# 294coder/Dif-PAN

Measured on AMD Instinct MI355X. Metric: fused megapixels/sec at T=1000, WV3 64x64x8 tiles, higher is better.
Workload: dtype f32-class (f16x2 split); 1 GPU; WV3 pansharpening, batch 64 of 64x64x8 tiles per GPU, T=1000 DDPM p_sample, fp32; tiles_per_gpu=64, tiles_total=64, T=1000, model_evaluations=1000, sampler=ddpm, parallelism=tile-shard x1, launches_per_denoising_step=132

## Files before the change

dif-pan_amd/csrc/ddif_dev.h:

```cpp
#pragma once
#include <hip/hip_runtime.h>

#ifdef DDIF_EMU
typedef hipemu_f32x16 f32x16;
typedef hipemu_f32x4 f32x4;
#define DDIF_MFMA_32x32x2(a, b, c) hipemu_mfma_32x32x2((a), (b), (c))
#define DDIF_MFMA_16x16x4(a, b, c) hipemu_mfma_16x16x4((a), (b), (c))
static inline f32x16 ddif_mfma_bf16_emu(float4 a, float4 b, f32x16 c) {
    hipemu_u32x4 ua, ub;
    __builtin_memcpy(&ua, &a, 16);
    __builtin_memcpy(&ub, &b, 16);
    return hipemu_mfma_32x32x16_bf16(ua, ub, c);
}
#define DDIF_MFMA_32x32x16_BF16(a, b, c) ddif_mfma_bf16_emu((a), (b), (c))
static inline f32x16 ddif_mfma_f16_emu(float4 a, float4 b, f32x16 c) {
    hipemu_u32x4 ua, ub;
    __builtin_memcpy(&ua, &a, 16);
    __builtin_memcpy(&ub, &b, 16);
    return hipemu_mfma_32x32x16_f16(ua, ub, c);
}
#define DDIF_MFMA_32x32x16_F16(a, b, c) ddif_mfma_f16_emu((a), (b), (c))
#define DDIF_DYN_SMEM(name) char* name = hipemu::tctx().dyn_smem
#define DDIF_SCHED_FENCE() ((void)0)
#else
// ... 103 lines not shown
#endif
__device__ __forceinline__ void dd_split2_pair(float a, float b, unsigned* hi, unsigned* lo) {
#ifdef DDIF_EMU
    const unsigned ha = dd_f16_bits(a), hb = dd_f16_bits(b);
    *hi = ha | (hb << 16);
    *lo = dd_f16_bits(a - dd_f16_val(ha)) | (dd_f16_bits(b - dd_f16_val(hb)) << 16);
#else
    typedef float v2f __attribute__((ext_vector_type(2)));
    typedef _Float16 v2h __attribute__((ext_vector_type(2)));
    const v2f v = {a, b};
    const v2h H = __builtin_convertvector(v, v2h);
    const v2f r = {a - (float)H.x, b - (float)H.y};
    *hi = __builtin_bit_cast(unsigned, H);
    *lo = __builtin_bit_cast(unsigned, __builtin_convertvector(r, v2h));
#endif
}
__device__ __forceinline__ float dd_silu_scaled(float x, float inv_s) {
#ifdef DDIF_EMU
    return x * (1.0f / fmaf(exp2f(-1.4426950408889634f * x), inv_s, inv_s));
#else
    return x * __builtin_amdgcn_rcpf(fmaf(__builtin_amdgcn_exp2f(-1.4426950408889634f * x), inv_s, inv_s));
#endif
}

__device__ __forceinline__ int dd_late(int v) {
#if !defined(DDIF_EMU) && defined(__HIP_DEVICE_COMPILE__)
    asm volatile("" : "+v"(v));
#endif
    return v;
}
// ... 144 lines not shown
```

dif-pan_amd/csrc/ddif_lr.cpp:

```cpp
#include "ddif_plan.h"
#include "kernels_lr.h"
#include "kernels_attn.h"

namespace ddif {

namespace {
template <int KS, int MB, int PRO, int EPI, bool F16 = false, bool B1 = false, bool ROWS = false>
ConvVariant lr_variant1(const char* name) {
    ConvVariant v;
    v.fn = conv_lr_kernel<KS, MB, PRO, EPI, 0, F16, B1, ROWS>;
    using G = LrGeom<KS, MB, PRO, (EPI & EPI_COLST) != 0, F16, B1>;
    v.smem = G::smem;
    v.th = G::TH;
    v.tw = G::TW;
    v.nt = 32;
    v.nthr = 256;
    v.x3 = true;
    v.f16 = F16;
    v.b1 = B1;
    v.lr = true;
    v.name = name;
    return v;
}
template <int MB, bool F16>
ConvVariant lr_rows_for(int pro, int epi) {
    if (pro == PRO_GN_SILU && epi == 0) return lr_variant1<3, MB, PRO_GN_SILU, 0, F16, false, true>("lr3x3_gn_silu_rows");
    if (pro == PRO_GN_SILU && epi == EPI_RES) return lr_variant1<3, MB, PRO_GN_SILU, EPI_RES, F16, false, true>("lr3x3_gn_silu_res_rows");
    if (pro == PRO_NONE && epi == EPI_SILU) return lr_variant1<3, MB, PRO_NONE, EPI_SILU, F16, false, true>("lr3x3_silu_rows");
    if (pro == PRO_NONE && epi == 0) return lr_variant1<3, MB, PRO_NONE, 0, F16, false, true>("lr3x3_rows");
    if (pro == PRO_NONE && epi == EPI_RES) return lr_variant1<3, MB, PRO_NONE, EPI_RES, F16, false, true>("lr3x3_res_rows");
    return ConvVariant();
}
template <int MB>
ConvVariant lr_for(int ks, int pro, int epi, int math) {
#define LRV(KS, PRO, EPI, NAME) (math == MATH_F16X2 ? lr_variant1<KS, MB, PRO, EPI, true>(NAME) : (math == MATH_BF16X1 ? lr_variant1<KS, MB, PRO, EPI, false, true>(NAME) : lr_variant1<KS, MB, PRO, EPI, false>(NAME)))
    if (ks == 3) {
        if (pro == PRO_GN_SILU && epi == 0) return LRV(3, PRO_GN_SILU, 0, "lr3x3_gn_silu");
        if (pro == PRO_GN_SILU && epi == EPI_RES) return LRV(3, PRO_GN_SILU, EPI_RES, "lr3x3_gn_silu_res");
        if (pro == PRO_NONE && epi == EPI_SILU) return LRV(3, PRO_NONE, EPI_SILU, "lr3x3_silu");
        if (pro == PRO_NONE && epi == 0) return LRV(3, PRO_NONE, 0, "lr3x3");
        if (pro == PRO_NONE && epi == EPI_RES) return LRV(3, PRO_NONE, EPI_RES, "lr3x3_res");
    } else if (ks == 1) {
        if (pro == PRO_NONE && epi == EPI_FILM) return LRV(1, PRO_NONE, EPI_FILM, "lr1x1_film");
        if (pro == PRO_NONE && epi == EPI_RES) return LRV(1, PRO_NONE, EPI_RES, "lr1x1_res");
        if (pro == PRO_NONE && epi == 0) return LRV(1, PRO_NONE, 0, "lr1x1");
        if (pro == PRO_NONE && epi == EPI_COLST) return LRV(1, PRO_NONE, EPI_COLST, "lr1x1_colstats");
        if (pro == PRO_GN && epi == 0) return LRV(1, PRO_GN, 0, "lr1x1_gn");
        if (pro == PRO_GN_SILU && epi == 0) return LRV(1, PRO_GN_SILU, 0, "lr1x1_gn_silu");
        if (pro == PRO_COLSM && epi == 0)
            return math == MATH_BF16X1 ? lr_variant1<1, MB, PRO_COLSM, 0, false, true>("lr1x1_colsoftmax") : lr_variant1<1, MB, PRO_COLSM, 0, false>("lr1x1_colsoftmax");
    }
// ... 46 lines not shown
```

dif-pan_amd/csrc/ddif_net.h:

```cpp
#pragma once
#include <mutex>
#include <cmath>
#include <cstdarg>
#include <cstdint>
#include <cstdio>
#include <cstring>
#include <functional>
#include <map>
#include <memory>
#include <string>
#include <vector>

#include "../../include/ddif.h"
#include "../../include/ddif_testops.h"
#include "ddif_dev.h"

namespace ddif {

extern thread_local std::string g_err;
int fail(int code, const char* fmt, ...);

#define DDIF_HIPCHK(x)                                                                                      \
    do {                                                                                                    \
        hipError_t e__ = (x);                                                                               \
        if (e__ != hipSuccess)                                                                              \
            return ::ddif::fail(DDIF_ERR_HIP, "%s failed: %s (%s:%d)", #x, hipGetErrorString(e__), __FILE__, \
                                __LINE__);                                                                  \
    } while (0)

enum { PRO_NONE = 0, PRO_GN = 1, PRO_GN_SILU = 2, PRO_COLSM = 3, PRO_GN_DW = 4 };

enum LayerKind { L_STEM, L_ENC, L_DOWN, L_MID, L_DEC, L_UP };

struct Layer {
    LayerKind kind;
    int cin = 0, cout = 0, cx = 0, cskip = 0;
    bool attn = false;
    std::string p;
};

struct PackedConv {
    const float* w = nullptr;
    const float* w_x3 = nullptr;
    const float* w_f16 = nullptr;
    const float* w_b1 = nullptr;
// ... 74 lines not shown
```

dif-pan_amd/csrc/ddif_plan.cpp:

```cpp
#include "ddif_plan.h"
#include <algorithm>
#include "kernels_conv.h"
#include "kernels_misc.h"
#include "attn_args.h"
#include "quantile_args.h"
#include "kernels_lafuse.h"

namespace ddif {

ConvVariant get_conv_variant(int ks, int stride, int ups, int ck, int pro, int cfg, int vec, int epi, int math) {
    if (cfg == 20 || cfg == 21)
        return (stride == 1 && !ups && vec == 1) ? get_lr_variant(ks, cfg == 20 ? 2 : 4, pro, epi, (math == MATH_F16X2 && pro == PRO_COLSM) ? MATH_BF16X3 : math) : ConvVariant();
    if (ks == 1) return get_conv_variant_k1(stride, ups, ck, pro, cfg, vec, epi);
    if (ks == 3) return epi ? get_conv_variant_k3e(stride, ups, ck, pro, cfg, vec, epi) : get_conv_variant_k3(stride, ups, ck, pro, cfg, vec);
    return ConvVariant();
}

static int num_cus();
static int x3_enabled() { static const int v = env_int("DDIF_X3", 1); return v; }
static int f16_enabled() { static const int v = env_int("DDIF_F16", 1); return v; }
int g_math_mode = [] { const char* e = getenv("DDIF_MATH"); return (e && std::strcmp(e, "bf16") == 0) ? 1 : 0; }();
int g_f16_raw = env_flag("DDIF_F16_RAW", true);
static int lr_rows_enabled() { static const int v = env_int("DDIF_LR_ROWS", 1); return v; }
static int lafuse_enabled() { static const int v = env_int("DDIF_LAFUSE", 1); return v; }
// ... 225 lines not shown
        allocs.push_back(q);
        bytes_allocated += arena_bytes;
        arena = reinterpret_cast<char*>(q);
    }
    if (int e = build_impl()) return e;
    if (arena_next != (int)lives.size()) return fail(DDIF_ERR_STATE, "plan arena: the two build passes disagree");
    return 0;
}

static int raise_dynamic_lds(ConvKernelFn fn, size_t var_smem) {
    if (var_smem + 8192 > 64 * 1024)
        DDIF_HIPCHK(hipFuncSetAttribute(reinterpret_cast<const void*>(fn), hipFuncAttributeMaxDynamicSharedMemorySize, (int)(var_smem + 8192)));
    return 0;
}

int Plan::add_conv(std::vector<Op>& prog, const ConvSpec& s, Tensor* out) {
    const PackedConv& pc = *s.pc;
    const int Hin = s.in0.H, Win = s.in0.W;
    const int Hc = s.ups ? 2 * Hin : Hin, Wc = s.ups ? 2 * Win : Win;
    const int Hout = s.stride == 2 ? (Hc - 1) / 2 + 1 : Hc, Wout = s.stride == 2 ? (Wc - 1) / 2 + 1 : Wc;
    const int c0 = s.in0.C, c1 = s.in1.C;
    if (c0 + c1 != pc.cin) return fail(DDIF_ERR_INVALID, "%s: input channels %d+%d != weight cin %d", s.name, c0, c1, pc.cin);
    if (pc.ks == 1 && (s.stride != 1 || s.ups)) return fail(DDIF_ERR_INVALID, "%s: 1x1 conv with stride/upsample", s.name);
    const int vec = (c0 % 4 != 0 || c1 % 4 != 0) ? 0 : ((c1 == 0 || c0 % pc.ck == 0) ? 1 : 2);
    if ((size_t)B * Hin * Win * (c0 > c1 ? c0 : c1) * 4 >= ((size_t)1 << 32) || (size_t)B * Hout * Wout * pc.cout * 8 >= ((size_t)1 << 32))
        return fail(DDIF_ERR_INVALID, "%s: a tensor of this batch reaches 4 GiB (32-bit offsets); split the batch", s.name);
    bool f16ok = f16_enabled() && !train_mode && pc.w_f16 && !s.w_override && !s.exact;
    const bool raw_in = !(s.pro == PRO_GN || s.pro == PRO_GN_SILU || s.pro == PRO_GN_DW);
    if (raw_in && !f16_raw) f16ok = false;
    if (f16ok && (s.pro == PRO_GN || s.pro == PRO_GN_SILU)) {
        auto ig = net->vec_absmax.find(s.gamma), ib = net->vec_absmax.find(s.beta);
// ... 31 lines not shown
    if (!var.fn && b1ok) {
        f16ok = f16ok0;
        choose(true, f16ok, false);
        var = variant(cfg, epi);
        general_kernel_if_no_lr(f16ok, false);
    }
    if (!var.fn) return fail(DDIF_ERR_INVALID, "%s: no kernel variant (ks=%d stride=%d ups=%d ck=%d pro=%d cfg=%d vec=%d epi=%d)", s.name, pc.ks, s.stride, s.ups, pc.ck, s.pro, cfg, vec, epi);
    bool lr_rows = false;
    if (var.lr && !var.b1 && pc.ks == 3 && Win == var.tw && Wout == Win && Hout == Hin && lr_rows_enabled()) {
        const ConvVariant vr = get_lr_variant(3, cfg == 20 ? 2 : 4, s.pro, epi, var.f16 ? MATH_F16X2 : MATH_BF16X3, true);
        if (vr.fn && vr.smem == var.smem) {
            var = vr;
            lr_rows = true;
        }
    }
    bool xf = false;
    if (s.xf && !train_mode && xf_enabled() && var.f16 && !var.lr && pc.ks == 3 && pc.cout == 32 && !s.ups && s.tb_off < 0 && !s.samp && s.xf->pc && s.xf->w && s.xf->film &&
        s.xf->pc->cin == 32 && s.xf->pc->bias && (s.xf->pc->cout == 32 || s.xf->pc->cout == 64) && &prog == &step) {
        const ConvVariant vx = get_xf_variant(s.stride, s.pro, cfg, vec, epi, s.xf->pc->cout / 32);
        if (vx.fn && vx.smem == var.smem) {
            var = vx;
            xf = true;
        }
    }
    if ((s.pro == PRO_GN || s.pro == PRO_GN_SILU || s.pro == PRO_GN_DW) && (!s.in0.st || (s.in1.p && !s.in1.st) || !s.gamma || !s.beta))
        return fail(DDIF_ERR_STATE, "%s: GroupNorm prologue without producer statistics", s.name);
    if (&prog == &step) {
        use(s.in0.p);
        use(s.in1.p);
        use(s.res);
// ... 103 lines not shown
        const ConvVariant vp = variant(cfg, EPI_SAMP | EPI_PRED);
        if (vp.fn && vp.smem == var.smem) {
            fn_samp_pred = vp.fn;
            if (int e = raise_dynamic_lds(fn_samp_pred, var.smem)) return e;
            final_fused_pred = true;
        }
    }
    const float* lms_p = lms.p;
    const bool dyn = s.dyn_input;
    const bool self_c = net->cfg.self_condition != 0;
    const int tb_off = s.tb_off;
    static const bool dump = getenv("DDIF_DUMP_PLAN") != nullptr;
    if (dump)
        fprintf(stderr, "[ddif plan] %-34s %-24s ks=%d s=%d u=%d  %3d+%3d -> %3d  @%3dx%-3d pro=%d epi=%d cfg=%d items=%ld grid=%u smem=%zu  in@%p out@%p\n", s.name, var.name, pc.ks, s.stride,
                s.ups, c0, c1, pc.cout, Hout, Wout, s.pro, epi, cfg, nwork, grid.x, smem, (const void*)s.in0.p, (const void*)out->p);
    Op op;
    op.name = var.name;
    {
        char lb[160];
        snprintf(lb, sizeof lb, "%s %dx%d %d+%d->%d @%dx%d cfg%d", s.name, pc.ks, pc.ks, c0, c1, pc.cout, Hout, Wout, cfg);
        op.label = lb;
    }
    op.flop = 2.0 * B * Hout * Wout * (double)pc.cout * (c0 + c1) * pc.ks * pc.ks;
    op.bytes = 4.0 * B * ((double)Hin * Win * (c0 + c1) + (double)Hout * Wout * pc.cout);
    if (xf) {
        op.label += " + x_conv+FiLM";
        op.flop += 2.0 * B * Hout * Wout * 32.0 * s.xf->pc->cout;
        op.bytes += 4.0 * B * (double)Hout * Wout * 3.0 * s.xf->pc->cout;
    }
    op.cls = (Hout * Wout <= 256) ? 2 : (pc.ks == 3 ? 0 : 1);
    op.mfma_w = var.b1 ? 1 : (var.f16 ? 3 : (var.x3 ? 6 : 16));
    op.timed = op.cls == 0;
    if (pc.ks == 3 && &prog == &step) {
        ++n_conv3;
        if (var.x3) ++n_conv3_x3;
        if (var.f16) ++n_conv3_f16;
// ... 886 lines not shown
        s.cs_mx = qmx;
        s.cs_sm = qsm;
        s.w_override = wmix;
        s.w_bstride = (long long)per;
        s.name = "softmax_H(q).ctx.attn_out+res";
        return p.add_conv(step, s, amix);
    }
    int ffn(const Dec& D, Tensor amix, Tensor* f3) {
        Tensor f1, f2;
        ConvSpec s;
        DDIF_TRY(need_conv(D.ci + ".ffn.0", &s.pc));
        s.in0 = amix;
        s.use_bias = false;
        s.silu = true;
        s.name = "ffn.0";
        DDIF_TRY(p.add_conv(step, s, &f1));
        ConvSpec s2;
        DDIF_TRY(need_conv(D.ci + ".ffn.2", &s2.pc));
        s2.in0 = f1;
        s2.use_bias = false;
        s2.name = "ffn.2";
        ConvSpec s3;
        DDIF_TRY(need_conv(D.ci + ".ffn.3", &s3.pc));
        if (const PackedConv* pm = PC(D.ci + ".ffn.23")) {
            ConvSpec sf = s2;
            sf.pc = pm;
            sf.use_bias = true;
            sf.res = amix.p;
            sf.stats = true;
            sf.name = "ffn.3(ffn.2) merged + res";
            return p.add_conv(step, sf, f3);
        }
        DDIF_TRY(p.add_conv(step, s2, &f2));
        s3.in0 = f2;
        s3.res = amix.p;
        s3.stats = true;
        s3.name = "ffn.3";
        return p.add_conv(step, s3, f3);
    }
    int decoder_block(const Layer& L) {
        Dec D;
        D.ci = L.p + ".cond_inj";
        D.skip = feats.back();
        feats.pop_back();
// ... 738 lines not shown
```

dif-pan_amd/csrc/ddif_plan.h:

```cpp
#pragma once
#include <cstdlib>
#include <string>
#include <memory>
#include "ddif_net.h"

namespace ddif {

inline int env_int(const char* name, int dflt) { const char* e = getenv(name); return e ? atoi(e) : dflt; }
inline bool env_flag(const char* name, bool dflt) { return env_int(name, dflt ? 1 : 0) != 0; }
bool train_x3();

struct ConvArgs;

struct Tensor {
    float* p = nullptr;
    int C = 0, H = 0, W = 0;
    double* st = nullptr;
    int np = 0;
};

struct StepCtx {
    const float* x = nullptr;
    const float* sc = nullptr;
    const float* tb = nullptr;
// ... 25 lines not shown
    int th = 0, tw = 0, nt = 0, nthr = 256;
    bool x3 = false;
    bool f16 = false;
    bool b1 = false;
    int wg_cap = 2;
    bool lr = false;
    bool wr = false;
    const char* name = "";
};
enum { MATH_BF16X3 = 0, MATH_F16X2 = 1, MATH_BF16X1 = 2 };
ConvVariant get_conv_variant(int ks, int stride, int ups, int ck, int pro, int cfg, int vec, int epi, int math = MATH_BF16X3);
ConvVariant get_lr_variant(int ks, int mb, int pro, int epi, int math = MATH_BF16X3, bool rows = false);
ConvVariant get_conv_variant_k1(int stride, int ups, int ck, int pro, int cfg, int vec, int epi);
ConvVariant get_conv_variant_k3(int stride, int ups, int ck, int pro, int cfg, int vec);
ConvVariant get_conv_variant_k3e(int stride, int ups, int ck, int pro, int cfg, int vec, int epi);
ConvVariant get_xf_variant(int stride, int pro, int cfg, int vec, int epi, int nbx);
extern int g_math_mode;
extern int g_f16_raw;
struct LaFuseArgs;
bool lafuse_supported(int H, int fea, int dout);
int lafuse_strip(int H, int nw = 8);
int lafuse_launch(const LaFuseArgs& a, int grid, hipStream_t s, bool prepare_only, int nw = 8);
bool lafuse8_supported(int H, int W, int c0, int c1, int dout);
int lafuse8_launch(const LaFuseArgs& a, int grid, hipStream_t s, bool prepare_only);
namespace tk {
void film_apply(hipStream_t s, const float* xc, const float* film, int B, int HW, int C, float* out, double* st_out, int chunks);
int film_chunks(int HW, int C);
size_t linattn_part_floats(int B, int H, int W, int C, int d);
void linattn_fwd(hipStream_t s, const float* q, const float* kv, int B, int heads, int d, int H, int W, float* out, int ld_o, float* ctx, float* part);
void linattn_ctx(hipStream_t s, const float* kv, int B, int heads, int d, int H, int W, float* ctx, float* part);
// ... 49 lines not shown
    int tb_off = -1;
    const float* res = nullptr;
    const float* film = nullptr;
    const float* w_override = nullptr;
    long long w_bstride = 0;
    const float* cs_mx = nullptr;
    const float* cs_sm = nullptr;
    const float* dw_w = nullptr;
    float* out_xn = nullptr;
    float* cso_mx = nullptr;
    float* cso_sm = nullptr;
    bool silu = false;
    bool stats = false;
    bool exact = false;
    bool samp = false;
    XfReq* xf = nullptr;
    const char* name = "conv";
};

struct Plan {
    Net* net = nullptr;
    unsigned long long generation = 0;
    int B = 0, H = 0, W = 0, C = 0, P = 0, CC = 0;
    std::vector<void*> allocs;
    std::vector<Op> pre, step;
    bool cond_set = false;
    bool train_mode = false;
    struct DropSite { float* mask; int C, H, W; };
    std::vector<DropSite> drop_sites;
    std::vector<float*> path_sites;
// ... 56 lines not shown
    char* arena = nullptr;
    size_t arena_bytes = 0, unaliased_bytes = 0;
    void use(const void* p);

    struct Tap { std::string name; Tensor t; int op; bool cond_only; };
    std::vector<Tap> taps;
    void tap(const std::string& name, const Tensor& t, bool cond_only = false);
    int forward_taps(const float* x, const float* t_host, const float* sc, float* out, int n, const int* ids, float* const* dst, hipStream_t s);
    ~Plan();
    int build();
    int build_impl();
    template <typename T>
    int dalloc(T** p, size_t n);
    int alloc_tensor(Tensor* t, int C, int H, int W, bool step_act = false);
    int add_conv(std::vector<Op>& prog, const ConvSpec& s, Tensor* out);
    int ensure_tb(int rows);
    int time_rows(const float* t_host, int rows, hipStream_t s);
    void run_prog(std::vector<Op>& prog, hipStream_t s, const StepCtx& ctx, bool prof);
    int n_conv3_f16 = 0;
    int n_conv3_b1 = 0;
    int n_conv3 = 0, n_conv3_x3 = 0;
    bool op_timing_done = false;

    struct TrainMod {
        enum Kind { STEM, FILM, RES, ATTN, DOWN, UP, DEC, FINAL } kind = STEM;
        std::string key;
        Tensor in, out;
        Tensor t[12];
        float* mask = nullptr;
        float* scale = nullptr;
// ... 60 lines not shown
```

dif-pan_amd/csrc/kernels_conv.h:

```cpp
#pragma once
#include "ddif_dev.h"
#include "sampler_dev.h"

namespace ddif {

struct ConvArgs {
    const float* in0;
    const float* in1;
    int c0, c1;
    int B, Hin, Win;
    int Hout, Wout, Cout;
    const float* w;
    int n_chunks;
    const float* bias;
    const float* tbias;
    int tbias_stride;
    const int* step_ptr;
    int tb_rowstride;
    const double* st0;
    int np0;
    const double* st1;
    int np1;
    const float* gamma;
    const float* beta;
// ... 24 lines not shown
    const float* xf_b;
    const float* xf_film;
    float* xf_out;
    double* xf_st;
    int xf_cout;
    int st_halves;
    int tiles_y8;
};

template <int F>
struct StageKind {
    static constexpr bool LAST = (F & 1) != 0;
    static constexpr bool TAIL = (F & 2) != 0;
};

enum { EPI_FILM = 1, EPI_SOUT = 2, EPI_RES = 4, EPI_SILU = 8, EPI_TBS = 16, EPI_COLST = 32, EPI_SAMP = 64, EPI_XF1 = 128, EPI_XF2 = 256, EPI_PRED = 512 };
template <int KS, int STRIDE, int UPS, int TH, int TW, int CK, int WM, int WN, int MB, int NB, int PRO, int VEC, int EPI = 0, int ABL = 0, int MATH = 0>
__global__ __launch_bounds__(64 * WM * WN) void conv_mfma_kernel(ConvArgs a) {
    constexpr int NW = WM * WN, NTHR = 64 * NW;
    constexpr int PAD = KS / 2;
    constexpr int IH = (TH - 1) * STRIDE + KS, IW = (TW - 1) * STRIDE + KS;
    constexpr bool X3 = MATH >= 1;
    constexpr bool F16 = MATH == 3 || MATH == 5;
    constexpr bool WR = MATH == 5;
    constexpr bool B1 = MATH == 4;
    constexpr int NPL = F16 ? 2 : (B1 ? 1 : 3);
    constexpr bool WSB = MATH == 2;
    constexpr int NWB = (WSB || WR) ? 1 : 2;
    constexpr int PS = CK / 2;
    constexpr int LDA = X3 ? NPL * PS + 4 : CK + 4;
    constexpr int LDH = CK + 4;
    constexpr int TAPS = KS * KS;
    constexpr int K8 = CK / 8;
    constexpr int K16 = CK / 16;
    constexpr int C4 = CK / 4;
    constexpr int NF = X3 ? TAPS * K16 : TAPS * K8;
    constexpr int RP = (X3 && KS == 3 && STRIDE == 1) ? (WR ? (64 - (IW * LDA) % 64) % 64 : (NPL == 2 ? 24 : (NPL == 1 ? 40 : 8))) : 0;
    constexpr int LDR = IW * LDA + RP;
    constexpr int ABUF = IH * LDR;
    constexpr bool DWM = (PRO == PRO_GN_DW);
    constexpr bool GNP = (PRO == PRO_GN || PRO == PRO_GN_SILU || PRO == PRO_GN_DW);
    constexpr bool FILM = (EPI & EPI_FILM) != 0, SOUT = (EPI & EPI_SOUT) != 0, RES = (EPI & EPI_RES) != 0, SILU = (EPI & EPI_SILU) != 0, TBS = (EPI & EPI_TBS) != 0;
    constexpr bool SAMP = (EPI & EPI_SAMP) != 0;
    constexpr bool PRED = (EPI & EPI_PRED) != 0;
    static_assert(!PRED || SAMP, "prediction conversion: sampler epilogue only");
    constexpr int NBX = (EPI & EPI_XF1) ? 1 : ((EPI & EPI_XF2) ? 2 : 0);
    constexpr bool XF = NBX > 0;
    static_assert(!SAMP || (!SOUT && !RES && !FILM), "sampler epilogue: the plain vector epilogue of the final conv");
    static_assert(!XF || (MB == 1 && NB == 1 && WN == 1 && !SOUT && !SAMP && !FILM && !SILU && PRO != PRO_GN_DW), "x_conv + FiLM fold: one wave holds all 32 couts of its pixels");
    static_assert(!DWM || (KS == 1 && STRIDE == 1 && !UPS && VEC == 1), "depthwise staging is for plain 1x1 convs");
    static_assert(PRO != PRO_COLSM || VEC == 1, "column-softmax prologue needs uniform-source float4 staging");
    constexpr int LPAD = DWM ? 1 : PAD;
    constexpr int LH = DWM ? TH + 2 : IH, LW = DWM ? TW + 2 : IW;
    constexpr int HBUF = DWM ? LH * LW * LDH : 0;
    constexpr int DWMAX = DWM ? 9 * 256 : 0;
    constexpr int DITEMS = (TH * TW * C4 + NTHR - 1) / NTHR;
// ... 250 lines not shown
        R.ok = l_ok;
        R.cb = cb;
        R.ch = l_ch;
        R.pos = L;
        if (++l_ch == a.n_chunks) {
            l_ch = 0;
            if (L.work + 1 < w1) {
                const bool same_tile = L.ct + 1 < a.n_ct;
                L = next_pos(L);
                if (!same_tile) item_geometry();
            }
        }
    };
    float fs_ga[4] = {0.f, 0.f, 0.f, 0.f}, fs_gb[4] = {0.f, 0.f, 0.f, 0.f};
    bool fs_colsm = false;
    constexpr bool RANGE = F16 && !GNP && !DWM;
    [[maybe_unused]] float r_max = 0.f;
    auto fs_begin = [&](StageRegs& R) {
        if (GNP) {
            if (R.pos.b != gn_b) {
                gn_finalize_wave(a.st0, a.np0, a.st1, a.np1, R.pos.b, (double)Ctot * a.Hin * a.Win, &mean, &rstd);
                gn_b = R.pos.b;
            }
            const float4 gq = *reinterpret_cast<const float4*>(&GBs[R.cb + c4 * 4]);
            const float4 bq = *reinterpret_cast<const float4*>(&GBs[GBN + R.cb + c4 * 4]);
#pragma unroll
            for (int i = 0; i < 4; ++i) {
                fs_ga[i] = (&gq.x)[i] * rstd;
                fs_gb[i] = (&bq.x)[i] - mean * fs_ga[i];
            }
        }
        fs_colsm = (PRO == PRO_COLSM) && R.cb < a.c0;
    };
    auto fs_item = [&](StageRegs& R, int buf, int it) {
        if ((ABL & 256) && R.sv[it].x != 12345.678f) return;
        float* dst = As + buf * ABUF;
        const bool ok = (R.ok >> it) & 1u;
        float v[4];
#pragma unroll
        for (int i = 0; i < 4; ++i) {
            float x = (&R.sv[it].x)[i];
            if (GNP) {
                x = fmaf(x, fs_ga[i], fs_gb[i]);
                if (PRO == PRO_GN_SILU) x = (F16 && !DWM) ? dd_silu_scaled(x, 1.0f / DDIF_F16_ASCALE) : dd_silu(x);
                else if (F16 && !DWM) x *= DDIF_F16_ASCALE;
            } else if (F16 && !DWM) {
                x *= DDIF_F16_ASCALE;
            }
            if (PRO == PRO_COLSM) {
                if (fs_colsm) x = dd_exp2_fast((x - (&R.mxv[it].x)[i]) * 1.4426950408889634f) * dd_rcp_fast((&R.smv[it].x)[i]);
            }
            v[i] = ok ? x : 0.f;
// ... 376 lines not shown
                                                const float mean = s_c0 * x0 + s_c1 * xi;
                                                o4[i] = mean + s_c2 * z;
                                            } else {
                                                const float eps = (s_c0 * xi - x0) / s_c1;
                                                float r = x0 * s_c2 + s_c3 * eps;
                                                if (s_c4 != 0.f) {
                                                    const float z = s_noise ? s_noise[e] : philox_normal(s_run.seed, (unsigned)(s_k + 1), (s_run.tile0 * a.Cout * hw) + e);
                                                    r += s_c4 * z;
                                                }
                                                o4[i] = r;
                                            }
                                        }
                                        *reinterpret_cast<float4*>(reinterpret_cast<char*>(a.s_out + tile_el) + (e_po[mb] + (unsigned)((nb * 32 + 8 * g) * 4))) = make_float4(o4[0], o4[1], o4[2], o4[3]);
                                    }
                                } else if (!GUARD || (e_pok[mb] && co < a.Cout)) {
                                    if (!(ABL & 4) || v[0] == 12345.678f)
                                        *reinterpret_cast<float4*>(obase + (e_po[mb] + (unsigned)((nb * 32 + 8 * g) * 4))) = make_float4(v[0], v[1], v[2], v[3]);
                                    s1 += (v[0] + v[1]) + (v[2] + v[3]);
                                    s2 += (v[0] * v[0] + v[1] * v[1]) + (v[2] * v[2] + v[3] * v[3]);
                                }
                            }
                    if constexpr (XF) {
                        char* xobase = reinterpret_cast<char*>(a.xf_out + (size_t)((Cp.b * a.Hout + Cp.oy0) * a.Wout + Cp.ox0) * (32 * NBX));
#pragma unroll
                        for (int nx = 0; nx < NBX; ++nx) {
                            f32x16 c2;
#pragma unroll
                            for (int r = 0; r < 16; ++r) c2[r] = 0.f;
#pragma unroll
                            for (int sx = 0; sx < 16; ++sx) c2 = DDIF_MFMA_32x32x2(xw[nx][sx], vx[sx], c2);
#pragma unroll
// ... 173 lines not shown
    }
#endif
    const int npairs = nflat >> 1;
    for (int pr = 0; pr < npairs; ++pr) {
        if (WR || bufch[0] == a.n_chunks - 1) stage(StageKind<1>{}, 0, R1, R0);
        else stage(StageKind<0>{}, 0, R1, R0);
        __syncthreads();
        if (WR || bufch[1] == a.n_chunks - 1) stage(StageKind<1>{}, 1, R0, R1);
        else stage(StageKind<0>{}, 1, R0, R1);
        __syncthreads();
    }
    if (nflat & 1) stage(StageKind<3>{}, 0, R1, R0);
    __syncthreads();
    flush_stats();
    stamp();
    if constexpr (RANGE) {
        if (a.range_flag && !(r_max < 65520.f)) *a.range_flag = 1;
    }
}


template <int KS, int STRIDE, int UPS, int TH, int TW, int CK, int NBT, int PRO = 0, int NW = 4, int MATH = 0>
constexpr size_t conv_smem_bytes() {
    constexpr int IH = (TH - 1) * STRIDE + KS, IW = (TW - 1) * STRIDE + KS;
    constexpr size_t dw = PRO == PRO_GN_DW ? (size_t)((TH + 2) * (TW + 2) * (CK + 4) + 9 * 256) : 0;
    constexpr int npl = (MATH == 3 || MATH == 5) ? 2 : (MATH == 4 ? 1 : 3);
    constexpr int lda = MATH >= 1 ? npl * CK / 2 + 4 : CK + 4, wchunk = MATH >= 1 ? KS * KS * (CK / 16) * npl * 256 : KS * KS * (CK / 8) * 256;
    constexpr int rp = (MATH >= 1 && KS == 3 && STRIDE == 1) ? (MATH == 5 ? (64 - (IW * lda) % 64) % 64 : (npl == 2 ? 24 : (npl == 1 ? 40 : 8))) : 0;
    return (size_t)(2 * IH * (IW * lda + rp) + ((MATH == 2 || MATH == 5) ? 1 : 2) * NBT * wchunk + dw) * sizeof(float) + 4 * NW * sizeof(double);
}
inline size_t conv_smem_extra(int pro, int n_chunks, int ck, int cout_pad, int xf_cout = 0) {
// ... 6 lines not shown
```

dif-pan_amd/csrc/kernels_lr.h:

```cpp
#pragma once
#include "kernels_conv.h"

namespace ddif {

#ifndef LR_ROWPAD
#define LR_ROWPAD 1
#endif
#if defined(DDIF_EMU) || !defined(__HIP_DEVICE_COMPILE__)
#define LR_PREFETCH_FENCE() ((void)0)
#elif defined(LR_NO_FENCE)
#define LR_PREFETCH_FENCE() ((void)0)
#else
#define LR_PREFETCH_FENCE() asm volatile("" ::: "memory")
#endif
template <int KS, int MB, int PRO, bool TALL = false, bool F16 = false, bool B1 = false>
struct LrGeom {
    static constexpr int NPL = F16 ? 2 : (B1 ? 1 : 3);
    static constexpr int TH = (TALL && MB == 4) ? 16 : 8, TW = (MB == 2 || TALL) ? 8 : 16;
    static constexpr int PAD = KS / 2;
    static constexpr int IH = TH + 2 * PAD, IW = TW + 2 * PAD;
    static constexpr int PC = (MB == 4 && KS == 3) ? 64 : 128;
    static constexpr int SP = PC / 16;
    static constexpr int APIX = SP * NPL * 8 + 4;
    static constexpr int RSL = (IW * APIX / 4) % 16;
// ... 7 lines not shown
    static constexpr int U = KS == 3 ? TAPS : SPW;
};

template <int KS, int MB, int PRO, int EPI, int ABL = 0, bool F16 = false, bool B1 = false, bool ROWS = false>
__global__ __launch_bounds__(256) void conv_lr_kernel(ConvArgs a) {
    constexpr bool COLST = (EPI & EPI_COLST) != 0;
    static_assert(!COLST || KS == 1, "column statistics epilogue: 1x1 convs");
    static_assert(!F16 || PRO != PRO_COLSM, "f16x2: the column-softmax prologue stays on bf16x3");
    static_assert(!(F16 && B1), "one operand format");
    using G = LrGeom<KS, MB, PRO, COLST, F16, B1>;
    constexpr int NPL = G::NPL, SLF = NPL * 8;
    constexpr int WSTEP = NPL * 1024;
    constexpr int TH = G::TH, TW = G::TW, LP = G::PAD, LH = G::IH, LW = G::IW, IW = G::IW, PC = G::PC, SP = G::SP;
    constexpr int APIX = G::APIX, AROW = G::AROW, TAPS = G::TAPS, U = G::U, SPW = G::SPW;
    constexpr bool GNP = (PRO == PRO_GN || PRO == PRO_GN_SILU);
    static_assert(PRO == PRO_NONE || PRO == PRO_GN || PRO == PRO_GN_SILU || PRO == PRO_COLSM, "prologues of the low-resolution kernel");
    constexpr bool FILM = (EPI & EPI_FILM) != 0, RES = (EPI & EPI_RES) != 0, SILU = (EPI & EPI_SILU) != 0;
    constexpr int C4 = PC / 4;
    constexpr int PSTEP = 256 / C4;
    constexpr int NIT = ROWS ? LH : (LH * LW + PSTEP - 1) / PSTEP;
    static_assert(256 % C4 == 0, "staging geometry");
    static_assert(!ROWS || (KS == 3 && PSTEP == TW && PRO != PRO_COLSM), "row staging: 3x3 convs, one pass of the threads = one image row");

    dd_touch_kernargs<sizeof(ConvArgs)>();
    DDIF_DYN_SMEM(smem);
    float* As = reinterpret_cast<float*>(smem);
    float* Red = As;
    float* Sst = As + (G::AFL > G::RFL ? G::AFL : G::RFL);

    const int tid = threadIdx.x, lane = tid & 63;
#ifdef DDIF_EMU
// ... 15 lines not shown
    const int NS = (Ctot + 15) / 16;
    const int NSW = a.n_chunks * (KS == 3 ? 1 : 2);
    const int NP = (NS + SP - 1) / SP;
    const int c4 = tid % C4, p0 = tid / C4;
    const int stepv = a.step_ptr ? *a.step_ptr : 0;

    int abase[MB];
#pragma unroll
    for (int mb = 0; mb < MB; ++mb) {
        const int m = mb * 32 + j;
        abase[mb] = (m / TW) * AROW + (m % TW) * APIX + 4 * h;
    }

    int gn_b = -1;
    float mean = 0.f, rstd = 1.f;
    constexpr bool RANGE = F16 && !GNP && PRO != PRO_COLSM;
    [[maybe_unused]] float r_max = 0.f;

    for (int work = w0; work < w1; ++work) {
        const int pt = work / a.n_ct, ct = work - pt * a.n_ct;
        const int bl = pt / tiles, t = pt - bl * tiles;
        const int b = a.b0 + bl;
        const int oy0 = (t / a.tiles_x) * TH, ox0 = (t % a.tiles_x) * TW;

        [[maybe_unused]] GnPartials gp;
        const bool new_b = GNP && b != gn_b;
        if (new_b) gn_load_partials(a.st0, a.np0, a.st1, a.np1, b, &gp);

        const int co = ct * 32 + 8 * wave + 4 * h;
        const bool cok_o = co < a.Cout;
        const int coc = cok_o ? co : 0;
// ... 97 lines not shown
                    }
                }
            }
#pragma unroll
            for (int it = 0; it < NIT; ++it) {
                const int pix = ROWS ? it * LW + p0 + LP : p0 + it * PSTEP;
                if constexpr (ROWS) {
                    if (!((okm >> it) & 1u)) {
                        float* d = &As[it * AROW + (p0 + LP) * APIX + slab_l * SLF + cin_slab / 2];
#pragma unroll
                        for (int q = 0; q < NPL; ++q) *reinterpret_cast<uint2*>(d + 8 * q) = make_uint2(0u, 0u);
                        continue;
                    }
                }
                const bool ok = ROWS ? cok : (okm >> it) & 1u;
                float v[4];
#pragma unroll
                for (int i = 0; i < 4; ++i) {
                    float x = (&sv[it].x)[i];
                    if constexpr (GNP) {
                        x = fmaf(x, ga[i], gb[i]);
                        if constexpr (PRO == PRO_GN_SILU) x = F16 ? dd_silu_scaled(x, 1.0f / DDIF_F16_ASCALE) : dd_silu(x);
                    } else if constexpr (F16) {
                        x *= DDIF_F16_ASCALE;
                    }
                    if constexpr (PRO == PRO_COLSM) {
                        if (colsm) x = dd_exp2_fast((x - (&mxv[it].x)[i]) * 1.4426950408889634f) * dd_rcp_fast((&smv[it].x)[i]);
                    }
                    v[i] = ok ? x : 0.f;
                }
// ... 115 lines not shown
            float v[4];
#pragma unroll
            for (int i = 0; i < 4; ++i) {
                float x = ((&pp[0].x)[i] + (&pp[1].x)[i]) + ((&pp[2].x)[i] + (&pp[3].x)[i]);
                x = F16 ? fmaf(x, DDIF_F16_OSCALE, (&bq.x)[i] + (&tq.x)[i]) : x + ((&bq.x)[i] + (&tq.x)[i]);
                if constexpr (FILM) x = x * (1.f + (&e_fs[mb].x)[i]) + (&e_fh[mb].x)[i];
                if constexpr (SILU) x = dd_silu(x);
                if constexpr (RES) x += (&e_res[mb].x)[i];
                v[i] = x;
            }
            if constexpr (COLST) {
#pragma unroll
                for (int i = 0; i < 4; ++i) colv[mb][i] = pok[mb] ? v[i] : -INFINITY;
            }
            if (pok[mb]) {
                if (!(ABL & 8) || v[0] == 12345.678f) *reinterpret_cast<float4*>(a.out + opix[mb] * a.Cout + co) = make_float4(v[0], v[1], v[2], v[3]);
                s1 += (v[0] + v[1]) + (v[2] + v[3]);
                s2 += (v[0] * v[0] + v[1] * v[1]) + (v[2] * v[2] + v[3] * v[3]);
            }
        }
        if constexpr (COLST) {
            float cm[4], cs[4];
#pragma unroll
            for (int i = 0; i < 4; ++i) {
                float m = colv[0][i];
#pragma unroll
                for (int mb = 1; mb < MB; ++mb) m = fmaxf(m, colv[mb][i]);
                m = fmaxf(m, __shfl_xor(m, 8));
                m = fmaxf(m, __shfl_xor(m, 16));
                float e = 0.f;
#pragma unroll
// ... 12 lines not shown
        }
        if (a.st_out) {
            const float t1 = wave_sum_fast(s1), t2 = wave_sum_fast(s2);
            if (lane == 63) {
                Sst[wave * 2 + 0] = t1;
                Sst[wave * 2 + 1] = t2;
            }
        }
        __syncthreads();
        if (a.st_out && tid == 0) {
            const size_t pi = ((size_t)b * (tiles * a.n_ct) + (size_t)t * a.n_ct + ct) * 2;
            a.st_out[pi + 0] = ((double)Sst[0] + (double)Sst[2]) + ((double)Sst[4] + (double)Sst[6]);
            a.st_out[pi + 1] = ((double)Sst[1] + (double)Sst[3]) + ((double)Sst[5] + (double)Sst[7]);
        }
    }
    if constexpr (RANGE) {
        if (a.range_flag && !(r_max < 65520.f)) *a.range_flag = 1;
    }
}

}
```

Measured before the change: 0.08414 MP/s.

## Hand off FFN intermediate as pre-split f16x2 planes between the two FFN convs

The first FFN conv (ffn.0, SiLU epilogue) now writes its output already scaled and split into f16 hi/lo planes. The following merged ffn.2/ffn.3 conv stages those planes into LDS with a plain copy instead of re-scaling and re-splitting each value in its prologue. This moves the f32-to-f16x2 conversion out of the consumer's staging path, where the halo causes it to be repeated, and does it once per element in the producer epilogue. It adds new kernel instantiations and couples the two convs' tile configs, and it only applies when both sides have matching variants.

```diff
diff --git a/dif-pan_amd/csrc/ddif_dev.h b/dif-pan_amd/csrc/ddif_dev.h
--- a/dif-pan_amd/csrc/ddif_dev.h
+++ b/dif-pan_amd/csrc/ddif_dev.h
@@ -141,6 +141,20 @@
     *hi = __builtin_bit_cast(unsigned, H);
     *lo = __builtin_bit_cast(unsigned, __builtin_convertvector(r, v2h));
 #endif
+}
+__device__ __forceinline__ uint4 dd_planes_quad(const float v[4], float* amax) {
+    const float s0 = v[0] * DDIF_F16_ASCALE, s1 = v[1] * DDIF_F16_ASCALE, s2 = v[2] * DDIF_F16_ASCALE, s3 = v[3] * DDIF_F16_ASCALE;
+    *amax = fmaxf(fmaxf(*amax, fmaxf(fabsf(s0), fabsf(s1))), fmaxf(fabsf(s2), fabsf(s3)));
+    uint4 q;
+    dd_split2_pair(s0, s1, &q.x, &q.z);
+    dd_split2_pair(s2, s3, &q.y, &q.w);
+    return q;
+}
+__device__ __forceinline__ float4 dd_bits_f4(const uint4& q) {
+    return make_float4(__builtin_bit_cast(float, q.x), __builtin_bit_cast(float, q.y), __builtin_bit_cast(float, q.z), __builtin_bit_cast(float, q.w));
+}
+__device__ __forceinline__ uint4 dd_f4_bits(const float4& f) {
+    return make_uint4(__builtin_bit_cast(unsigned, f.x), __builtin_bit_cast(unsigned, f.y), __builtin_bit_cast(unsigned, f.z), __builtin_bit_cast(unsigned, f.w));
 }
 __device__ __forceinline__ float dd_silu_scaled(float x, float inv_s) {
 #ifdef DDIF_EMU
diff --git a/dif-pan_amd/csrc/ddif_lr.cpp b/dif-pan_amd/csrc/ddif_lr.cpp
--- a/dif-pan_amd/csrc/ddif_lr.cpp
+++ b/dif-pan_amd/csrc/ddif_lr.cpp
@@ -29,12 +29,18 @@
     if (pro == PRO_NONE && epi == EPI_SILU) return lr_variant1<3, MB, PRO_NONE, EPI_SILU, F16, false, true>("lr3x3_silu_rows");
     if (pro == PRO_NONE && epi == 0) return lr_variant1<3, MB, PRO_NONE, 0, F16, false, true>("lr3x3_rows");
     if (pro == PRO_NONE && epi == EPI_RES) return lr_variant1<3, MB, PRO_NONE, EPI_RES, F16, false, true>("lr3x3_res_rows");
+    if constexpr (F16) {
+        if (pro == PRO_NONE && epi == (EPI_SILU | EPI_PLANES)) return lr_variant1<3, MB, PRO_NONE, EPI_SILU | EPI_PLANES, true, false, true>("lr3x3_silu_rows");
+        if (pro == PRO_PLANES && epi == EPI_RES) return lr_variant1<3, MB, PRO_PLANES, EPI_RES, true, false, true>("lr3x3_res_rows");
+    }
     return ConvVariant();
 }
 template <int MB>
 ConvVariant lr_for(int ks, int pro, int epi, int math) {
 #define LRV(KS, PRO, EPI, NAME) (math == MATH_F16X2 ? lr_variant1<KS, MB, PRO, EPI, true>(NAME) : (math == MATH_BF16X1 ? lr_variant1<KS, MB, PRO, EPI, false, true>(NAME) : lr_variant1<KS, MB, PRO, EPI, false>(NAME)))
     if (ks == 3) {
+        if (pro == PRO_NONE && epi == (EPI_SILU | EPI_PLANES)) return math == MATH_F16X2 ? lr_variant1<3, MB, PRO_NONE, EPI_SILU | EPI_PLANES, true>("lr3x3_silu") : ConvVariant();
+        if (pro == PRO_PLANES && epi == EPI_RES) return math == MATH_F16X2 ? lr_variant1<3, MB, PRO_PLANES, EPI_RES, true>("lr3x3_res") : ConvVariant();
         if (pro == PRO_GN_SILU && epi == 0) return LRV(3, PRO_GN_SILU, 0, "lr3x3_gn_silu");
         if (pro == PRO_GN_SILU && epi == EPI_RES) return LRV(3, PRO_GN_SILU, EPI_RES, "lr3x3_gn_silu_res");
         if (pro == PRO_NONE && epi == EPI_SILU) return LRV(3, PRO_NONE, EPI_SILU, "lr3x3_silu");
diff --git a/dif-pan_amd/csrc/ddif_net.h b/dif-pan_amd/csrc/ddif_net.h
--- a/dif-pan_amd/csrc/ddif_net.h
+++ b/dif-pan_amd/csrc/ddif_net.h
@@ -28,7 +28,7 @@
                                 __LINE__);                                                                  \
     } while (0)
 
-enum { PRO_NONE = 0, PRO_GN = 1, PRO_GN_SILU = 2, PRO_COLSM = 3, PRO_GN_DW = 4 };
+enum { PRO_NONE = 0, PRO_GN = 1, PRO_GN_SILU = 2, PRO_COLSM = 3, PRO_GN_DW = 4, PRO_PLANES = 5 };
 
 enum LayerKind { L_STEM, L_ENC, L_DOWN, L_MID, L_DEC, L_UP };
 
diff --git a/dif-pan_amd/csrc/ddif_plan.cpp b/dif-pan_amd/csrc/ddif_plan.cpp
--- a/dif-pan_amd/csrc/ddif_plan.cpp
+++ b/dif-pan_amd/csrc/ddif_plan.cpp
@@ -263,7 +263,13 @@
     return 0;
 }
 
-int Plan::add_conv(std::vector<Op>& prog, const ConvSpec& s, Tensor* out) {
+struct Plan::ConvSel {
+    ConvVariant var;
+    int cfg = 0, math = MATH_BF16X3, epi = 0, vec = 0;
+    bool lr_rows = false, raw_in = false;
+    bool planes = false;
+};
+int Plan::select_conv(const ConvSpec& s, ConvSel* sel) {
     const PackedConv& pc = *s.pc;
     const int Hin = s.in0.H, Win = s.in0.W;
     const int Hc = s.ups ? 2 * Hin : Hin, Wc = s.ups ? 2 * Win : Win;
@@ -325,6 +331,49 @@
             lr_rows = true;
         }
     }
+    bool planes = false;
+    if ((s.planes_out || s.planes_in) && var.f16 && !var.wr && !b1ok && !s.film && !s.cso_mx && s.tb_off < 0 && !s.samp && !s.xf && !s.in1.p && s.pro == PRO_NONE) {
+        const int ppro = s.planes_in ? PRO_PLANES : s.pro, pepi = epi | (s.planes_out ? EPI_PLANES : 0);
+        const ConvVariant vp = var.lr ? get_lr_variant(3, cfg == 20 ? 2 : 4, ppro, pepi, MATH_F16X2, lr_rows) : get_planes_variant(s.stride, s.ups, pc.ck, ppro, cfg, vec, pepi);
+        if (pc.ks == 3 && vp.fn && vp.smem == var.smem && vp.th == var.th && vp.tw == var.tw && vp.nt == var.nt && vp.nthr == var.nthr) {
+            var = vp;
+            planes = true;
+        }
+    }
+    sel->var = var;
+    sel->cfg = cfg;
+    sel->math = math;
+    sel->epi = epi;
+    sel->vec = vec;
+    sel->lr_rows = lr_rows;
+    sel->raw_in = raw_in;
+    sel->planes = planes;
+    return 0;
+}
+
+static const int g_ffn_planes = env_int("DDIF_FFN_PLANES", 7);
+bool Plan::conv_takes_planes(const ConvSpec& s) {
+    ConvSel sel;
+    const std::string saved = g_err;
+    const bool ok = select_conv(s, &sel) == 0 && sel.planes && (g_ffn_planes & (!sel.var.lr ? 1 : (sel.cfg == 21 ? 2 : 4))) != 0;
+    g_err = saved;
+    return ok;
+}
+
+int Plan::add_conv(std::vector<Op>& prog, const ConvSpec& s, Tensor* out) {
+    const PackedConv& pc = *s.pc;
+    const int Hin = s.in0.H, Win = s.in0.W;
+    const int Hc = s.ups ? 2 * Hin : Hin, Wc = s.ups ? 2 * Win : Win;
+    const int Hout = s.stride == 2 ? (Hc - 1) / 2 + 1 : Hc, Wout = s.stride == 2 ? (Wc - 1) / 2 + 1 : Wc;
+    const int c0 = s.in0.C, c1 = s.in1.C;
+    ConvSel sel;
+    if (int e = select_conv(s, &sel)) return e;
+    const int vec = sel.vec;
+    if ((s.planes_out || s.planes_in) && !sel.planes) return fail(DDIF_ERR_STATE, "%s: f16x2 planes asked for, but the chosen tiling has no such instantiation", s.name);
+    ConvVariant var = sel.var;
+    const int cfg = sel.cfg, math = sel.math, epi = sel.epi;
+    const bool lr_rows = sel.lr_rows, raw_in = sel.raw_in;
+    auto variant = [&](int cfg_, int epi_) { return get_conv_variant(pc.ks, s.stride, s.ups, pc.ck, s.pro, cfg_, vec, epi_, math); };
     bool xf = false;
     if (s.xf && !train_mode && xf_enabled() && var.f16 && !var.lr && pc.ks == 3 && pc.cout == 32 && !s.ups && s.tb_off < 0 && !s.samp && s.xf->pc && s.xf->w && s.xf->film &&
         s.xf->pc->cin == 32 && s.xf->pc->bias && (s.xf->pc->cout == 32 || s.xf->pc->cout == 64) && &prog == &step) {
@@ -458,12 +507,14 @@
     if (dump)
         fprintf(stderr, "[ddif plan] %-34s %-24s ks=%d s=%d u=%d  %3d+%3d -> %3d  @%3dx%-3d pro=%d epi=%d cfg=%d items=%ld grid=%u smem=%zu  in@%p out@%p\n", s.name, var.name, pc.ks, s.stride,
                 s.ups, c0, c1, pc.cout, Hout, Wout, s.pro, epi, cfg, nwork, grid.x, smem, (const void*)s.in0.p, (const void*)out->p);
+    if (dump && sel.planes) fprintf(stderr, "[ddif ffn-planes] %-34s %-24s cfg=%d %s\n", s.name, var.name, cfg, s.planes_out ? "writes f16x2 planes" : "stages f16x2 planes by copy");
     Op op;
     op.name = var.name;
     {
         char lb[160];
         snprintf(lb, sizeof lb, "%s %dx%d %d+%d->%d @%dx%d cfg%d", s.name, pc.ks, pc.ks, c0, c1, pc.cout, Hout, Wout, cfg);
         op.label = lb;
+        if (sel.planes) op.label += s.planes_out ? " planes-out" : " planes-in";
     }
     op.flop = 2.0 * B * Hout * Wout * (double)pc.cout * (c0 + c1) * pc.ks * pc.ks;
     op.bytes = 4.0 * B * ((double)Hin * Win * (c0 + c1) + (double)Hout * Wout * pc.cout);
@@ -1380,6 +1431,20 @@
         s.use_bias = false;
         s.silu = true;
         s.name = "ffn.0";
+        bool planes = false;
+        if (const PackedConv* pm = train ? nullptr : PC(D.ci + ".ffn.23")) {
+            ConvSpec a = s, b;
+            a.planes_out = true;
+            b.pc = pm;
+            b.in0.C = s.pc->cout;
+            b.in0.H = amix.H;
+            b.in0.W = amix.W;
+            b.res = amix.p;
+            b.stats = true;
+            b.planes_in = true;
+            planes = pm->cin == s.pc->cout && p.conv_takes_planes(a) && p.conv_takes_planes(b);
+        }
+        s.planes_out = planes;
         DDIF_TRY(p.add_conv(step, s, &f1));
         ConvSpec s2;
         DDIF_TRY(need_conv(D.ci + ".ffn.2", &s2.pc));
@@ -1394,6 +1459,7 @@
             sf.use_bias = true;
             sf.res = amix.p;
             sf.stats = true;
+            sf.planes_in = planes;
             sf.name = "ffn.3(ffn.2) merged + res";
             return p.add_conv(step, sf, f3);
         }
diff --git a/dif-pan_amd/csrc/ddif_plan.h b/dif-pan_amd/csrc/ddif_plan.h
--- a/dif-pan_amd/csrc/ddif_plan.h
+++ b/dif-pan_amd/csrc/ddif_plan.h
@@ -63,6 +63,7 @@
 ConvVariant get_conv_variant_k1(int stride, int ups, int ck, int pro, int cfg, int vec, int epi);
 ConvVariant get_conv_variant_k3(int stride, int ups, int ck, int pro, int cfg, int vec);
 ConvVariant get_conv_variant_k3e(int stride, int ups, int ck, int pro, int cfg, int vec, int epi);
+ConvVariant get_planes_variant(int stride, int ups, int ck, int pro, int cfg, int vec, int epi);
 ConvVariant get_xf_variant(int stride, int pro, int cfg, int vec, int epi, int nbx);
 extern int g_math_mode;
 extern int g_f16_raw;
@@ -142,6 +143,8 @@
     bool stats = false;
     bool exact = false;
     bool samp = false;
+    bool planes_out = false;
+    bool planes_in = false;
     XfReq* xf = nullptr;
     const char* name = "conv";
 };
@@ -228,6 +231,9 @@
     int dalloc(T** p, size_t n);
     int alloc_tensor(Tensor* t, int C, int H, int W, bool step_act = false);
     int add_conv(std::vector<Op>& prog, const ConvSpec& s, Tensor* out);
+    struct ConvSel;
+    int select_conv(const ConvSpec& s, ConvSel* sel);
+    bool conv_takes_planes(const ConvSpec& s);
     int ensure_tb(int rows);
     int time_rows(const float* t_host, int rows, hipStream_t s);
     void run_prog(std::vector<Op>& prog, hipStream_t s, const StepCtx& ctx, bool prof);
diff --git a/dif-pan_amd/csrc/ddif_planes.cpp b/dif-pan_amd/csrc/ddif_planes.cpp
--- /dev/null
+++ b/dif-pan_amd/csrc/ddif_planes.cpp
@@ -0,0 +1,35 @@
+#include "ddif_plan.h"
+#include "kernels_conv.h"
+
+namespace ddif {
+
+namespace {
+template <int TH, int TW, int NW, int PRO, int EPI>
+ConvVariant pl1(const char* name) {
+    ConvVariant v;
+    v.fn = conv_mfma_kernel<3, 1, 0, TH, TW, 16, NW, 1, 1, 1, PRO, 1, EPI, 0, 3>;
+    v.smem = conv_smem_bytes<3, 1, 0, TH, TW, 16, 1, PRO, NW, 3>();
+    v.th = TH;
+    v.tw = TW;
+    v.nt = 32;
+    v.nthr = 64 * NW;
+    v.x3 = v.f16 = true;
+    v.name = name;
+    return v;
+}
+}
+
+ConvVariant get_planes_variant(int stride, int ups, int ck, int pro, int cfg, int vec, int epi) {
+    if (stride != 1 || ups || ck != 16 || vec != 1) return ConvVariant();
+    if (pro == PRO_NONE && epi == (EPI_SILU | EPI_PLANES)) {
+        if (cfg == 27) return pl1<16, 16, 8, PRO_NONE, EPI_SILU | EPI_PLANES>("conv3x3_silu");
+        if (cfg == 28) return pl1<8, 16, 4, PRO_NONE, EPI_SILU | EPI_PLANES>("conv3x3_silu");
+    }
+    if (pro == PRO_PLANES && epi == EPI_RES) {
+        if (cfg == 27) return pl1<16, 16, 8, PRO_PLANES, EPI_RES>("conv3x3_res");
+        if (cfg == 28) return pl1<8, 16, 4, PRO_PLANES, EPI_RES>("conv3x3_res");
+    }
+    return ConvVariant();
+}
+
+}
diff --git a/dif-pan_amd/csrc/kernels_conv.h b/dif-pan_amd/csrc/kernels_conv.h
--- a/dif-pan_amd/csrc/kernels_conv.h
+++ b/dif-pan_amd/csrc/kernels_conv.h
@@ -62,7 +62,7 @@
     static constexpr bool TAIL = (F & 2) != 0;
 };
 
-enum { EPI_FILM = 1, EPI_SOUT = 2, EPI_RES = 4, EPI_SILU = 8, EPI_TBS = 16, EPI_COLST = 32, EPI_SAMP = 64, EPI_XF1 = 128, EPI_XF2 = 256, EPI_PRED = 512 };
+enum { EPI_FILM = 1, EPI_SOUT = 2, EPI_RES = 4, EPI_SILU = 8, EPI_TBS = 16, EPI_COLST = 32, EPI_SAMP = 64, EPI_XF1 = 128, EPI_XF2 = 256, EPI_PRED = 512, EPI_PLANES = 1024 };
 template <int KS, int STRIDE, int UPS, int TH, int TW, int CK, int WM, int WN, int MB, int NB, int PRO, int VEC, int EPI = 0, int ABL = 0, int MATH = 0>
 __global__ __launch_bounds__(64 * WM * WN) void conv_mfma_kernel(ConvArgs a) {
     constexpr int NW = WM * WN, NTHR = 64 * NW;
@@ -88,6 +88,10 @@
     constexpr int ABUF = IH * LDR;
     constexpr bool DWM = (PRO == PRO_GN_DW);
     constexpr bool GNP = (PRO == PRO_GN || PRO == PRO_GN_SILU || PRO == PRO_GN_DW);
+    constexpr bool PLN_IN = (PRO == PRO_PLANES);
+    constexpr bool PLN_OUT = (EPI & EPI_PLANES) != 0;
+    static_assert(!PLN_IN || (F16 && VEC == 1), "planes input: f16x2 instantiations with float4 staging");
+    static_assert(!PLN_OUT || !(EPI & (EPI_SOUT | EPI_SAMP | EPI_XF1 | EPI_XF2)), "planes output: the plain vector epilogue");
     constexpr bool FILM = (EPI & EPI_FILM) != 0, SOUT = (EPI & EPI_SOUT) != 0, RES = (EPI & EPI_RES) != 0, SILU = (EPI & EPI_SILU) != 0, TBS = (EPI & EPI_TBS) != 0;
     constexpr bool SAMP = (EPI & EPI_SAMP) != 0;
     constexpr bool PRED = (EPI & EPI_PRED) != 0;
@@ -368,7 +372,7 @@
     };
     float fs_ga[4] = {0.f, 0.f, 0.f, 0.f}, fs_gb[4] = {0.f, 0.f, 0.f, 0.f};
     bool fs_colsm = false;
-    constexpr bool RANGE = F16 && !GNP && !DWM;
+    constexpr bool RANGE = F16 && !GNP && !DWM && !PLN_IN;
     [[maybe_unused]] float r_max = 0.f;
     auto fs_begin = [&](StageRegs& R) {
         if (GNP) {
@@ -390,6 +394,13 @@
         if ((ABL & 256) && R.sv[it].x != 12345.678f) return;
         float* dst = As + buf * ABUF;
         const bool ok = (R.ok >> it) & 1u;
+        if constexpr (PLN_IN) {
+            const uint4 q = dd_f4_bits(R.sv[it]);
+            const int ps = ((a_in >> it) & 1u) ? PS : 0;
+            *reinterpret_cast<uint2*>(&dst[a_lds[it]]) = make_uint2(ok ? q.x : 0u, ok ? q.y : 0u);
+            *reinterpret_cast<uint2*>(&dst[a_lds[it] + ps]) = make_uint2(ok ? q.z : 0u, ok ? q.w : 0u);
+            return;
+        }
         float v[4];
 #pragma unroll
         for (int i = 0; i < 4; ++i) {
@@ -796,7 +807,9 @@
                                         *reinterpret_cast<float4*>(reinterpret_cast<char*>(a.s_out + tile_el) + (e_po[mb] + (unsigned)((nb * 32 + 8 * g) * 4))) = make_float4(o4[0], o4[1], o4[2], o4[3]);
                                     }
                                 } else if (!GUARD || (e_pok[mb] && co < a.Cout)) {
-                                    if (!(ABL & 4) || v[0] == 12345.678f)
+                                    if constexpr (PLN_OUT)
+                                        *reinterpret_cast<float4*>(obase + (e_po[mb] + (unsigned)((nb * 32 + 8 * g) * 4))) = dd_bits_f4(dd_planes_quad(v, &r_max));
+                                    else if (!(ABL & 4) || v[0] == 12345.678f)
                                         *reinterpret_cast<float4*>(obase + (e_po[mb] + (unsigned)((nb * 32 + 8 * g) * 4))) = make_float4(v[0], v[1], v[2], v[3]);
                                     s1 += (v[0] + v[1]) + (v[2] + v[3]);
                                     s2 += (v[0] * v[0] + v[1] * v[1]) + (v[2] * v[2] + v[3] * v[3]);
@@ -1000,7 +1013,7 @@
     __syncthreads();
     flush_stats();
     stamp();
-    if constexpr (RANGE) {
+    if constexpr (RANGE || PLN_OUT) {
         if (a.range_flag && !(r_max < 65520.f)) *a.range_flag = 1;
     }
 }
diff --git a/dif-pan_amd/csrc/kernels_lr.h b/dif-pan_amd/csrc/kernels_lr.h
--- a/dif-pan_amd/csrc/kernels_lr.h
+++ b/dif-pan_amd/csrc/kernels_lr.h
@@ -45,7 +45,10 @@
     constexpr int TH = G::TH, TW = G::TW, LP = G::PAD, LH = G::IH, LW = G::IW, IW = G::IW, PC = G::PC, SP = G::SP;
     constexpr int APIX = G::APIX, AROW = G::AROW, TAPS = G::TAPS, U = G::U, SPW = G::SPW;
     constexpr bool GNP = (PRO == PRO_GN || PRO == PRO_GN_SILU);
-    static_assert(PRO == PRO_NONE || PRO == PRO_GN || PRO == PRO_GN_SILU || PRO == PRO_COLSM, "prologues of the low-resolution kernel");
+    constexpr bool PLN_IN = (PRO == PRO_PLANES), PLN_OUT = (EPI & EPI_PLANES) != 0;
+    static_assert(PRO == PRO_NONE || PRO == PRO_GN || PRO == PRO_GN_SILU || PRO == PRO_COLSM || PRO == PRO_PLANES, "prologues of the low-resolution kernel");
+    static_assert(!PLN_IN || F16, "planes input: f16x2 instantiations");
+    static_assert(!PLN_OUT || !COLST, "planes output: plain epilogues");
     constexpr bool FILM = (EPI & EPI_FILM) != 0, RES = (EPI & EPI_RES) != 0, SILU = (EPI & EPI_SILU) != 0;
     constexpr int C4 = PC / 4;
     constexpr int PSTEP = 256 / C4;
@@ -91,7 +94,7 @@
 
     int gn_b = -1;
     float mean = 0.f, rstd = 1.f;
-    constexpr bool RANGE = F16 && !GNP && PRO != PRO_COLSM;
+    constexpr bool RANGE = F16 && !GNP && PRO != PRO_COLSM && !PLN_IN;
     [[maybe_unused]] float r_max = 0.f;
 
     for (int work = w0; work < w1; ++work) {
@@ -219,6 +222,15 @@
                     }
                 }
                 const bool ok = ROWS ? cok : (okm >> it) & 1u;
+                if constexpr (PLN_IN) {
+                    if (ROWS || pix < LH * LW) {
+                        float* d = ROWS ? &As[it * AROW + (p0 + LP) * APIX + slab_l * SLF + cin_slab / 2] : &As[(pix / LW) * AROW + (pix % LW) * APIX + slab_l * SLF + cin_slab / 2];
+                        const uint4 q = dd_f4_bits(sv[it]);
+                        *reinterpret_cast<uint2*>(d) = make_uint2(ok ? q.x : 0u, ok ? q.y : 0u);
+                        *reinterpret_cast<uint2*>(d + 8) = make_uint2(ok ? q.z : 0u, ok ? q.w : 0u);
+                    }
+                    continue;
+                }
                 float v[4];
 #pragma unroll
                 for (int i = 0; i < 4; ++i) {
@@ -364,7 +376,8 @@
                 for (int i = 0; i < 4; ++i) colv[mb][i] = pok[mb] ? v[i] : -INFINITY;
             }
             if (pok[mb]) {
-                if (!(ABL & 8) || v[0] == 12345.678f) *reinterpret_cast<float4*>(a.out + opix[mb] * a.Cout + co) = make_float4(v[0], v[1], v[2], v[3]);
+                if constexpr (PLN_OUT) *reinterpret_cast<float4*>(a.out + opix[mb] * a.Cout + co) = dd_bits_f4(dd_planes_quad(v, &r_max));
+                else if (!(ABL & 8) || v[0] == 12345.678f) *reinterpret_cast<float4*>(a.out + opix[mb] * a.Cout + co) = make_float4(v[0], v[1], v[2], v[3]);
                 s1 += (v[0] + v[1]) + (v[2] + v[3]);
                 s2 += (v[0] * v[0] + v[1] * v[1]) + (v[2] * v[2] + v[3] * v[3]);
             }
@@ -407,7 +420,7 @@
             a.st_out[pi + 1] = ((double)Sst[1] + (double)Sst[3]) + ((double)Sst[5] + (double)Sst[7]);
         }
     }
-    if constexpr (RANGE) {
+    if constexpr (RANGE || PLN_OUT) {
         if (a.range_flag && !(r_max < 65520.f)) *a.range_flag = 1;
     }
 }
```

Result: no change. 0.08451 MP/s, median of 6 (+0.4%).
